# lidongyv/Explicit-Context-Mapping-for-Stereo-Matching

Measured on AMD Instinct MI355X. Metric: stereo-pairs/sec (cmfsm train step fwd+bwd+Adam), higher is better.
Workload: dtype f32; 1 GPU; SceneFlow 960x540 (padded to 576) D=192 batch=4/GPU fwd+bwd+Adam (train.py path); arch=cmfsm, global_batch=4, parallelism=dp1, cost_volume=collapsed into class-indexed 2-D convolutions, launch=eager

## Files before the change

### explicit-context-mapping-for-stereo-matching_amd/csrc/conv3d_wgrad.hip

```cpp
#include "common.h"

#ifdef WG_PROFILE
__device__ unsigned long long wg_prof[4 * 8];
#define WG_T(i) do { const unsigned long long now_ = clock64(); prof[i] += now_ - last; last = now_; } while (0)
#else
#define WG_T(i) do { } while (0)
#endif

namespace {

typedef float f32x16 __attribute__((ext_vector_type(16)));

constexpr int CT = 32;
constexpr int TWV = 16;

template <int STRIDE, int TD, int TH, int KD, int KH = 3, int KW = 3, int DIL = 1>
struct WgCfg {
    static_assert(KD == 1 || (KH == 3 && KW == 3 && DIL == 1), "3-D layers are 3x3x3, dilation 1");
    static constexpr int NTAPS = KH * KW * KD, PADD = KD / 2;
    static constexpr int TG = NTAPS >= 15 ? 4 : NTAPS >= 2 ? 2 : 1, KG = 4 / TG, MAXNT = (NTAPS + TG - 1) / TG;
    static constexpr int ID = (TD - 1) * STRIDE + KD, IH = (TH - 1) * STRIDE + (KH - 1) * DIL + 1,
                         IW = (TWV - 1) * STRIDE + (KW - 1) * DIL + 1;
    static constexpr int RS = IW;
    static constexpr int XCH = ID * IH * RS;
    static constexpr int XSTR = (XCH % 2 == 0) ? XCH + 1 : XCH + 2;
    static constexpr int NV = TD * TH * TWV;
    static constexpr int GSTR = NV + 1;
    static constexpr int LDS_FLOATS = CT * XSTR + CT * GSTR;
    static constexpr int LDS_BYTES = LDS_FLOATS * 4;
};


template <int STRIDE, int TD, int TH, int KD, int KH, int KW, int DIL, int TGI, int KGI, int NLOADS, class Issue>
__device__ __forceinline__ void wg_tile(const float* __restrict__ ga, const float* __restrict__ xb,
                                        f32x16 (&acc)[WgCfg<STRIDE, TD, TH, KD, KH, KW, DIL>::MAXNT], Issue&& issue) {
    using Cfg = WgCfg<STRIDE, TD, TH, KD, KH, KW, DIL>;
    constexpr int IH = Cfg::IH, RS = Cfg::RS;
    constexpr int T0 = TGI * Cfg::MAXNT;
    constexpr int NT = (T0 + Cfg::MAXNT <= Cfg::NTAPS) ? Cfg::MAXNT : Cfg::NTAPS - T0;
    static_assert(NT >= 1, "every wave owns at least one tap");
    constexpr int KSA = TD * TH * TWV / 2;
    constexpr int KS0 = KGI * (KSA / Cfg::KG), KS = KS0 + KSA / Cfg::KG;
    constexpr int KSI = (KS - KS0) * 3 / 4;
    constexpr int LPK = (NLOADS + KSI - 1) / KSI;
    auto b_off = [](int ks, int t) constexpr {
        const int xx = (ks * 2) % TWV, hy = ((ks * 2) / TWV) % TH, dz = (ks * 2) / (TWV * TH);
        const int tap = T0 + t, kd = KD == 3 ? tap / 9 : 0, kh = (tap / KW) % KH, kw = tap % KW;
        return ((dz * STRIDE + kd) * IH + hy * STRIDE + kh * DIL) * RS + xx * STRIDE + kw * DIL;
    };
    float a_cur = ga[KS0 * 2], b_cur[NT];
#pragma unroll
    for (int t = 0; t < NT; ++t) b_cur[t] = xb[b_off(KS0, t)];
#pragma unroll
    for (int ks = KS0; ks < KS; ++ks) {
        float a_nxt = 0.f, b_nxt[NT];
        if (ks + 1 < KS) {
            a_nxt = ga[(ks + 1) * 2];
#pragma unroll
            for (int t = 0; t < NT; ++t) b_nxt[t] = xb[b_off(ks + 1, t)];
        }
#pragma unroll
        for (int q = 0; q < LPK; ++q)
            if ((ks - KS0) * LPK + q < NLOADS) issue((ks - KS0) * LPK + q);
#pragma unroll
        for (int t = 0; t < NT; ++t) acc[t] = __builtin_amdgcn_mfma_f32_32x32x2f32(a_cur, b_cur[t], acc[t], 0, 0, 0);
        __builtin_amdgcn_sched_barrier(0);
        a_cur = a_nxt;
#pragma unroll
        for (int t = 0; t < NT; ++t) b_cur[t] = b_nxt[t];
    }
}

template <int TD, int TH, int KD, int I, int NLOADS, class Issue>
__device__ __forceinline__ void wg_tile_wino(const float* __restrict__ gaw, const float* __restrict__ xbw,
                                             f32x16 (&acc)[4 * KD], Issue&& issue) {
    using Cfg = WgCfg<1, TD, TH, KD>;
    constexpr int IH = Cfg::IH, RS = Cfg::RS, NP = TD + KD - 1;
    constexpr int PAIRS = TWV / 4, KS = (TH / 2) * PAIRS;
    constexpr int RA = I == 0 ? 0 : I == 2 ? 2 : 1, RB = I == 0 ? 2 : I == 1 ? 2 : I == 2 ? 1 : 3;
    float xr_[NP][2][4], gr_[TD][2][2];
    float bq[NP][4], aq[TD][4];
    auto read_raw = [&](int ks) {
        const int tr = ks / PAIRS, pr = ks % PAIRS;
        const float* xk = xbw + 2 * tr * RS + 4 * pr;
        const float* gk = gaw + 2 * tr * TWV + 4 * pr;
#pragma unroll
        for (int p = 0; p < NP; ++p)
#pragma unroll
            for (int j = 0; j < 4; ++j) {
                xr_[p][0][j] = xk[(p * IH + RA) * RS + j];
                xr_[p][1][j] = xk[(p * IH + RB) * RS + j];
            }
#pragma unroll
        for (int d = 0; d < TD; ++d)
#pragma unroll
            for (int r = 0; r < 2; ++r)
#pragma unroll
                for (int c = 0; c < 2; ++c) gr_[d][r][c] = gk[(d * TH + r) * TWV + c];
    };
    auto make_operands = [&]() {
#pragma unroll
        for (int p = 0; p < NP; ++p) {
            float e[4];
#pragma unroll
            for (int j = 0; j < 4; ++j) e[j] = I == 1 ? xr_[p][0][j] + xr_[p][1][j] : xr_[p][0][j] - xr_[p][1][j];
            bq[p][0] = e[0] - e[2]; bq[p][1] = e[1] + e[2]; bq[p][2] = e[2] - e[1]; bq[p][3] = e[1] - e[3];
        }
#pragma unroll
        for (int d = 0; d < TD; ++d) {
            float m[2];
#pragma unroll
            for (int c = 0; c < 2; ++c)
                m[c] = I == 0 ? gr_[d][0][c] : I == 1 ? gr_[d][0][c] + gr_[d][1][c]
                     : I == 2 ? gr_[d][0][c] - gr_[d][1][c] : -gr_[d][1][c];
            aq[d][0] = m[0]; aq[d][1] = m[0] + m[1]; aq[d][2] = m[0] - m[1]; aq[d][3] = -m[1];
        }
    };
    constexpr int NPH = KD == 1 ? 16 : 8, KPP = KS / NPH, LPP = (NLOADS + NPH - 2) / (NPH - 1);
    constexpr int KUNROLL = KD == 1 ? 8 : 1;
    static_assert(KS % NPH == 0, "k-steps split into phases");
    read_raw(0);
    make_operands();
#pragma unroll
    for (int ph = 0; ph < NPH; ++ph) {
        if (ph < NPH - 1) {
#pragma unroll
            for (int q = 0; q < LPP; ++q)
                if (ph * LPP + q < NLOADS) issue(ph * LPP + q);
        }
#pragma unroll KUNROLL
        for (int ks = ph * KPP; ks < (ph + 1) * KPP; ++ks) {
            if (ks + 1 < KS) read_raw(ks + 1);
            __builtin_amdgcn_sched_barrier(0);
#pragma unroll
            for (int j = 0; j < 4; ++j)
#pragma unroll
                for (int kd = 0; kd < KD; ++kd)
#pragma unroll
                    for (int d = 0; d < TD; ++d)
                        acc[j * KD + kd] = __builtin_amdgcn_mfma_f32_32x32x2f32(aq[d][j], bq[d + kd][j], acc[j * KD + kd], 0, 0, 0);
            __builtin_amdgcn_sched_barrier(0);
            if (ks + 1 < KS) make_operands();
            __builtin_amdgcn_sched_barrier(0);
        }
    }
}

template <int STRIDE, int TD, int TH, int KD, int KH = 3, int KW = 3, int DIL = 1, bool WINO = false>
__global__ __launch_bounds__(256, KD == 3 ? 1 : 2) void conv3d_wgrad_mfma(const float* __restrict__ x, const float* __restrict__ gy,
                                                         float* __restrict__ partial, int B, int Ci, int Co, int D,
                                                         int H, int W, int Do, int Ho, int Wo, int tiles_d, int tiles_h,
                                                         int tiles_w, int ci_tiles, int pad_top, int pad_left) {
    using Cfg = WgCfg<STRIDE, TD, TH, KD, KH, KW, DIL>;
    constexpr int ID = Cfg::ID, IH = Cfg::IH, IW = Cfg::IW, XSTR = Cfg::XSTR, NV = Cfg::NV, GSTR = Cfg::GSTR,
                  NTAPS = Cfg::NTAPS, MAXNT = Cfg::MAXNT;
    extern __shared__ __attribute__((aligned(16))) float smem[];
    float* Xs = smem;
    float* Gs = smem + CT * XSTR;

    const int tid = threadIdx.x, lane = tid & 63, wave = tid >> 6;
    const int l31 = lane & 31, half = lane >> 5;
    const int ci0 = (blockIdx.y % ci_tiles) * CT, co0 = (blockIdx.y / ci_tiles) * CT;
    const int tgi = wave % Cfg::TG, kgi = wave / Cfg::TG;
    const int t0 = tgi * MAXNT;
    constexpr int NACC = WINO ? 4 * KD : MAXNT;
    static_assert(!WINO || (STRIDE == 1 && KH == 3 && KW == 3 && DIL == 1 && TH % 2 == 0), "Winograd form: 3x3, stride 1");
    f32x16 acc[NACC];
#pragma unroll
    for (int t = 0; t < NACC; ++t)
#pragma unroll
        for (int i = 0; i < 16; ++i) acc[t][i] = 0.f;

    const size_t HWi = (size_t)H * W, DHWi = (size_t)D * HWi;
    const size_t HWo = (size_t)Ho * Wo, DHWo = (size_t)Do * HWo;
    const int ntiles = B * tiles_d * tiles_h * tiles_w;

    constexpr int NPOSX = ID * IH * IW;
    constexpr int PPX = (NPOSX + 255) / 256;
    constexpr int GPL = 256 / NV;
    static_assert(256 % NV == 0 && CT % GPL == 0, "gy tile must divide the workgroup");
    constexpr int NGRP = CT / GPL;
    constexpr int NLOADS = CT * PPX + NGRP;
    float xr[CT * PPX], gr[NGRP];
    const unsigned xplane = (unsigned)DHWi * 4u, gplane = (unsigned)DHWo * 4u;
    const int nci = Ci - ci0 < CT ? Ci - ci0 : CT, nco = Co - co0 < CT ? Co - co0 : CT;
    unsigned xoff[PPX], goff;
    auto xrs = __builtin_amdgcn_make_buffer_rsrc(const_cast<float*>(x), 0, 0, 0x00020000);
    auto grs = xrs;
    int pdz[PPX], phy[PPX], pxx[PPX], prel[PPX];
#pragma unroll
    for (int j = 0; j < PPX; ++j) {
        int t = tid + j * 256;
        pxx[j] = t % IW; t /= IW;
        phy[j] = t % IH;
        const bool in_tile = tid + j * 256 < NPOSX;
        prel[j] = in_tile ? (t / IH) * (int)HWi + phy[j] * W + pxx[j] : 0;
        pdz[j] = in_tile ? t / IH : -(1 << 20);
    }
    const int gv = tid % NV, gccl = tid / NV;
    const int gxx = gv % TWV, ghy = (gv / TWV) % TH, gdz = gv / (TWV * TH);
    const int grel = gdz * (int)HWo + ghy * Wo + gxx;
    auto prefetch_setup = [&](unsigned tile) {
        const bool live = tile < (unsigned)ntiles;
        unsigned r = live ? tile : 0u;
        const int td = (int)(r % (unsigned)tiles_d); r /= (unsigned)tiles_d;
        const int tw = (int)(r % (unsigned)tiles_w); r /= (unsigned)tiles_w;
        const int th = (int)(r % (unsigned)tiles_h);
        const int b = (int)(r / (unsigned)tiles_h);
        const int od0 = td * TD, oh0 = th * TH, ow0 = tw * TWV;
        const int id0 = od0 * STRIDE - Cfg::PADD, ih0 = oh0 * STRIDE - pad_top, iw0 = ow0 * STRIDE - pad_left;
        const int xbase = id0 * (int)HWi + ih0 * W + iw0;
#pragma unroll
        for (int j = 0; j < PPX; ++j) {
            const bool ok = live && (unsigned)(id0 + pdz[j]) < (unsigned)D && (unsigned)(ih0 + phy[j]) < (unsigned)H &&
                            (unsigned)(iw0 + pxx[j]) < (unsigned)W;
            xoff[j] = ok ? (unsigned)(xbase + prel[j]) * 4u : 0x80000000u;
        }
        xrs = __builtin_amdgcn_make_buffer_rsrc(const_cast<float*>(x + ((size_t)b * Ci + ci0) * DHWi), 0,
                                                (unsigned)nci * xplane, 0x00020000);
        const bool vok = live && od0 + gdz < Do && oh0 + ghy < Ho && ow0 + gxx < Wo;
        goff = vok ? (unsigned)(od0 * (int)HWo + oh0 * Wo + ow0 + grel) * 4u + (unsigned)gccl * gplane : 0x80000000u;
        grs = __builtin_amdgcn_make_buffer_rsrc(const_cast<float*>(gy + ((size_t)b * Co + co0) * DHWo), 0,
                                                (unsigned)nco * gplane, 0x00020000);
    };
    auto prefetch_issue = [&](int i) {
        if (i < CT * PPX) {
            const int cc = i / PPX, j = i % PPX;
            xr[i] = __builtin_bit_cast(float, __builtin_amdgcn_raw_buffer_load_b32(xrs, xoff[j] + (unsigned)cc * xplane, 0, 0));
        } else {
            const int g = i - CT * PPX;
            gr[g] = __builtin_bit_cast(float, __builtin_amdgcn_raw_buffer_load_b32(grs, goff + (unsigned)(g * GPL) * gplane, 0, 0));
        }
    };
#ifdef WG_PROFILE
    unsigned long long prof[8] = {0, 0, 0, 0, 0, 0, 0, 0}, last = clock64();
#endif
    unsigned tile0 = blockIdx.x, tile_end = (unsigned)ntiles, tile_step = gridDim.x;
    if ((gridDim.x & 7u) == 0u) {
        const unsigned xcd = blockIdx.x & 7u, q = (unsigned)ntiles >> 3, rr = (unsigned)ntiles & 7u;
        const unsigned start = xcd * q + (xcd < rr ? xcd : rr);
        tile0 = start + (blockIdx.x >> 3);
        tile_end = start + q + (xcd < rr ? 1u : 0u);
        tile_step = gridDim.x >> 3;
    }
    prefetch_setup(tile0 < tile_end ? tile0 : (unsigned)ntiles);
#pragma unroll
    for (int i = 0; i < NLOADS; ++i) prefetch_issue(i);
    WG_T(0);
    for (unsigned tile = tile0; tile < tile_end; tile += tile_step) {
        __syncthreads();
        WG_T(1);
#pragma unroll
        for (int j = 0; j < PPX; ++j) {
            const int p = tid + j * 256 < NPOSX ? tid + j * 256 : NPOSX;
#pragma unroll
            for (int cc = 0; cc < CT; ++cc) Xs[cc * XSTR + p] = xr[cc * PPX + j];
        }
#pragma unroll
        for (int g = 0; g < NGRP; ++g) Gs[(g * GPL + tid / NV) * GSTR + tid % NV] = gr[g];
        WG_T(2);
        __syncthreads();
        WG_T(3);
        prefetch_setup(tile + tile_step < tile_end ? tile + tile_step : (unsigned)ntiles);
        WG_T(4);
        if constexpr (WINO) {
            const float* gaw = Gs + l31 * GSTR + half * 2;
            const float* xbw = Xs + l31 * XSTR + half * 2;
            switch (wave) {
                case 0: wg_tile_wino<TD, TH, KD, 0, NLOADS>(gaw, xbw, acc, prefetch_issue); break;
                case 1: wg_tile_wino<TD, TH, KD, 1, NLOADS>(gaw, xbw, acc, prefetch_issue); break;
                case 2: wg_tile_wino<TD, TH, KD, 2, NLOADS>(gaw, xbw, acc, prefetch_issue); break;
                default: wg_tile_wino<TD, TH, KD, 3, NLOADS>(gaw, xbw, acc, prefetch_issue); break;
            }
        } else {
        const float* ga = Gs + l31 * GSTR + half;
        const float* xb = Xs + l31 * XSTR + half * STRIDE;
        switch (wave) {
            case 0: wg_tile<STRIDE, TD, TH, KD, KH, KW, DIL, 0 % Cfg::TG, 0 / Cfg::TG, NLOADS>(ga, xb, acc, prefetch_issue); break;
            case 1: wg_tile<STRIDE, TD, TH, KD, KH, KW, DIL, 1 % Cfg::TG, 1 / Cfg::TG, NLOADS>(ga, xb, acc, prefetch_issue); break;
            case 2: wg_tile<STRIDE, TD, TH, KD, KH, KW, DIL, 2 % Cfg::TG, 2 / Cfg::TG, NLOADS>(ga, xb, acc, prefetch_issue); break;
            default: wg_tile<STRIDE, TD, TH, KD, KH, KW, DIL, 3 % Cfg::TG, 3 / Cfg::TG, NLOADS>(ga, xb, acc, prefetch_issue); break;
        }
        }
        WG_T(5);
    }
#ifdef WG_PROFILE
    if (blockIdx.x == 0 && blockIdx.y == 0 && lane == 0)
        for (int i = 0; i < 8; ++i) wg_prof[wave * 8 + i] = prof[i];
#endif
    if constexpr (WINO) {
        float* pw = partial + (size_t)blockIdx.x * 16 * KD * Co * Ci;
        const int ci = ci0 + l31;
#pragma unroll
        for (int t = 0; t < NACC; ++t) {
            const int j = t / KD, kd = t % KD;
#pragma unroll
            for (int i = 0; i < 16; ++i) {
                const int co = co0 + mfma32_row(i, half);
                if (co < Co && ci < Ci) pw[((size_t)((wave * 4 + j) * KD + kd) * Co + co) * Ci + ci] = acc[t][i];
            }
        }
        return;
    }
    float* pp = partial + ((size_t)blockIdx.x * Cfg::KG + kgi) * Co * Ci * NTAPS;
#pragma unroll
    for (int t = 0; t < MAXNT; ++t) {
        const int tap = t0 + t;
        if (tap >= NTAPS) continue;
        const int ci = ci0 + l31;
#pragma unroll
        for (int i = 0; i < 16; ++i) {
            const int co = co0 + mfma32_row(i, half);
            if (co < Co && ci < Ci) pp[((size_t)co * Ci + ci) * NTAPS + tap] = acc[t][i];
        }
    }
}

__global__ __launch_bounds__(256) void wgrad_reduce(const float* __restrict__ partial, float* __restrict__ gw, int n, int P) {
    __shared__ float sm[8][32];
    const int o = threadIdx.x & 31, grp = threadIdx.x >> 5;
    const int i = blockIdx.x * 32 + o;
    float s = 0.f;
    if (i < n) {
        float s0 = 0.f, s1 = 0.f, s2 = 0.f, s3 = 0.f;
        int p = grp;
        for (; p + 24 < P; p += 32) {
            s0 += partial[(size_t)p * n + i];
            s1 += partial[(size_t)(p + 8) * n + i];
            s2 += partial[(size_t)(p + 16) * n + i];
            s3 += partial[(size_t)(p + 24) * n + i];
        }
        for (; p < P; p += 8) s0 += partial[(size_t)p * n + i];
        s = (s0 + s1) + (s2 + s3);
    }
    sm[grp][o] = s;
    __syncthreads();
    if (grp == 0 && i < n) {
        float t = 0.f;
#pragma unroll
        for (int g = 0; g < 8; ++g) t += sm[g][o];
        gw[i] = t;
    }
}

__global__ void wgrad_wino_finish(const float* __restrict__ gU, float* __restrict__ gw, int Co, int Ci, int KD) {
    const int idx = blockIdx.x * blockDim.x + threadIdx.x;
    if (idx >= Co * Ci * KD) return;
    const int kd = idx % KD, ci = (idx / KD) % Ci, co = idx / (KD * Ci);
    float u[4][4];
#pragma unroll
    for (int i = 0; i < 4; ++i)
#pragma unroll
        for (int j = 0; j < 4; ++j) u[i][j] = gU[((size_t)((i * 4 + j) * KD + kd) * Co + co) * Ci + ci];
    float t[3][4];
#pragma unroll
    for (int j = 0; j < 4; ++j) {
        t[0][j] = u[0][j] + 0.5f * (u[1][j] + u[2][j]);
        t[1][j] = 0.5f * (u[1][j] - u[2][j]);
        t[2][j] = 0.5f * (u[1][j] + u[2][j]) + u[3][j];
    }
    float* o = gw + (((size_t)co * Ci + ci) * KD + kd) * 9;
#pragma unroll
    for (int a = 0; a < 3; ++a) {
        o[a * 3 + 0] = t[a][0] + 0.5f * (t[a][1] + t[a][2]);
        o[a * 3 + 1] = 0.5f * (t[a][1] - t[a][2]);
        o[a * 3 + 2] = 0.5f * (t[a][1] + t[a][2]) + t[a][3];
    }
}

inline int wgrad_workers(int Ci, int Co, long long ntiles, int occ = 1) {
    const int ytiles = ((Ci + CT - 1) / CT) * ((Co + CT - 1) / CT);
    long long p = 256 * occ / ytiles;
    if (p < 1) p = 1;
    if (p > ntiles) p = ntiles;
    return (int)p;
}

template <int STRIDE, int TD, int TH, int KD, int KH = 3, int KW = 3, int DIL = 1>
int launch_wgrad(const float* x, const float* gy, float* gw, float* partial, int B, int Ci, int Co, int D, int H, int W,
                 hipStream_t st, int Ho = 0, int Wo = 0, int pad_top = 1, int pad_left = 1) {
    using Cfg = WgCfg<STRIDE, TD, TH, KD, KH, KW, DIL>;
    const int Do = (D - 1) / STRIDE + 1;
    if (Ho <= 0) Ho = (H - 1) / STRIDE + 1;
    if (Wo <= 0) Wo = (W - 1) / STRIDE + 1;
    const int tiles_d = (Do + TD - 1) / TD, tiles_h = (Ho + TH - 1) / TH, tiles_w = (Wo + TWV - 1) / TWV;
    const long long ntiles = (long long)B * tiles_d * tiles_h * tiles_w;
    const int ci_tiles = (Ci + CT - 1) / CT, co_tiles = (Co + CT - 1) / CT;
    const int P = wgrad_workers(Ci, Co, ntiles, KD == 3 ? 1 : 2);
    auto kern = conv3d_wgrad_mfma<STRIDE, TD, TH, KD, KH, KW, DIL>;
    {
        const hipError_t e = ecm_allow_lds(reinterpret_cast<const void*>(kern), Cfg::LDS_BYTES);
        if (e != hipSuccess) return (int)e;
    }
    hipLaunchKernelGGL(kern, dim3(P, ci_tiles * co_tiles), dim3(256), Cfg::LDS_BYTES, st, x, gy, partial, B, Ci, Co, D, H,
                       W, Do, Ho, Wo, tiles_d, tiles_h, tiles_w, ci_tiles, pad_top, pad_left);
    const int n = Co * Ci * Cfg::NTAPS;
    hipLaunchKernelGGL(wgrad_reduce, dim3((n + 31) / 32), dim3(256), 0, st, partial, gw, n, P * Cfg::KG);
    return ECM_LAUNCH_RESULT();
}

template <int TD, int TH, int KD>
int launch_wgrad_wino(const float* x, const float* gy, float* gw, float* scratch, int B, int Ci, int Co, int D, int H, int W,
                      hipStream_t st) {
    using Cfg = WgCfg<1, TD, TH, KD>;
    const int tiles_d = (D + TD - 1) / TD, tiles_h = (H + TH - 1) / TH, tiles_w = (W + TWV - 1) / TWV;
    const long long ntiles = (long long)B * tiles_d * tiles_h * tiles_w;
    const int ci_tiles = (Ci + CT - 1) / CT, co_tiles = (Co + CT - 1) / CT;
    const int P = wgrad_workers(Ci, Co, ntiles, KD == 3 ? 1 : 2);
    auto kern = conv3d_wgrad_mfma<1, TD, TH, KD, 3, 3, 1, true>;
    {
        const hipError_t e = ecm_allow_lds(reinterpret_cast<const void*>(kern), Cfg::LDS_BYTES);
        if (e != hipSuccess) return (int)e;
    }
    const int n = 16 * KD * Co * Ci;
    float* partial = scratch;
    float* gU = scratch + (size_t)P * n;
    hipLaunchKernelGGL(kern, dim3(P, ci_tiles * co_tiles), dim3(256), Cfg::LDS_BYTES, st, x, gy, partial, B, Ci, Co, D, H,
                       W, D, H, W, tiles_d, tiles_h, tiles_w, ci_tiles, 1, 1);
    hipLaunchKernelGGL(wgrad_reduce, dim3((n + 31) / 32), dim3(256), 0, st, partial, gU, n, P);
    hipLaunchKernelGGL(wgrad_wino_finish, dim3((Co * Ci * KD + 255) / 256), dim3(256), 0, st, gU, gw, Co, Ci, KD);
    return ECM_LAUNCH_RESULT();
}

inline long long ntiles_wino(int B, int D, int H, int W, int kd) {
    const int TD = kd == 3 ? 2 : 1, TH = kd == 3 ? 8 : 16;
    return (long long)B * ((D + TD - 1) / TD) * ((H + TH - 1) / TH) * ((W + TWV - 1) / TWV);
}

inline long long ntiles_for(int B, int D, int H, int W, int stride) {
    const int Do = (D - 1) / stride + 1, Ho = (H - 1) / stride + 1, Wo = (W - 1) / stride + 1;
    const int TD = stride == 1 ? 2 : 1, TH = stride == 1 ? 8 : 4;
    return (long long)B * ((Do + TD - 1) / TD) * ((Ho + TH - 1) / TH) * ((Wo + TWV - 1) / TWV);
}

}

extern "C" long long ecm_conv3d_wgrad_scratch_bytes(int B, int Ci, int Co, int D, int H, int W, int stride) {
    if (B <= 0 || Ci <= 0 || Co <= 0 || D <= 0 || H <= 0 || W <= 0 || (stride != 1 && stride != 2)) return 0;
    return (long long)wgrad_workers(Ci, Co, ntiles_for(B, D, H, W, stride)) * Co * Ci * 27 * (long long)sizeof(float);
}

extern "C" int ecm_conv3d_k3_wgrad(const float* x, const float* gy, float* gw, void* scratch, long long scratch_bytes,
                                   int B, int Ci, int Co, int D, int H, int W, int stride, void* stream) {
    ECM_CHECK_ARG(x && gy && gw && scratch && B > 0 && Ci > 0 && Co > 0 && D > 0 && H > 0 && W > 0);
    if (stride != 1 && stride != 2) return ECM_EUNSUP;
    if ((long long)D * H * W * 4 * 32 >= 0x7fffffffLL) return ECM_EUNSUP;
    if (ntiles_for(B, D, H, W, stride) >= 0x7fffffffLL) return ECM_EUNSUP;
    if (scratch_bytes < ecm_conv3d_wgrad_scratch_bytes(B, Ci, Co, D, H, W, stride)) return ECM_ESCRATCH;
    float* partial = static_cast<float*>(scratch);
    hipStream_t st = ecm_stream(stream);
    if (stride == 1) return launch_wgrad<1, 2, 8, 3>(x, gy, gw, partial, B, Ci, Co, D, H, W, st);
    return launch_wgrad<2, 1, 4, 3>(x, gy, gw, partial, B, Ci, Co, D, H, W, st);
}

namespace {
inline long long ntiles2d_ex(int B, int Ho, int Wo, int stride) {
    const int th = stride == 1 ? 16 : 8;
    return (long long)B * ((Ho + th - 1) / th) * ((Wo + TWV - 1) / TWV);
}
}

extern "C" long long ecm_conv2d_wgrad_ex_scratch_bytes(int B, int Ci, int Co, int Ho, int Wo, int kh, int kw, int stride) {
    if (B <= 0 || Ci <= 0 || Co <= 0 || Ho <= 0 || Wo <= 0 || kh <= 0 || kw <= 0) return 0;
    return (long long)wgrad_workers(Ci, Co, ntiles2d_ex(B, Ho, Wo, stride), 2) * 4 * Co * Ci * kh * kw * (long long)sizeof(float);
}

extern "C" int ecm_conv2d_wgrad_ex(const float* x, const float* gy, float* gw, void* scratch, long long scratch_bytes, int B,
                                   int Ci, int Co, int H, int W, int kh, int kw, int stride, int dil, int pad_top,
                                   int pad_left, int Ho, int Wo, void* stream) {
    ECM_CHECK_ARG(x && gy && gw && scratch && B > 0 && Ci > 0 && Co > 0 && H > 0 && W > 0 && Ho > 0 && Wo > 0);
    if ((long long)H * W * 4 * 32 >= 0x7fffffffLL || (long long)Ho * Wo * 4 * 32 >= 0x7fffffffLL) return ECM_EUNSUP;
    if (ntiles2d_ex(B, Ho, Wo, stride) >= 0x7fffffffLL) return ECM_EUNSUP;
    if (scratch_bytes < ecm_conv2d_wgrad_ex_scratch_bytes(B, Ci, Co, Ho, Wo, kh, kw, stride)) return ECM_ESCRATCH;
    float* partial = static_cast<float*>(scratch);
    hipStream_t st = ecm_stream(stream);
#define WG2(KH, KW, S, DL, TH) if (kh == KH && kw == KW && stride == S && dil == DL) \
        return launch_wgrad<S, 1, TH, 1, KH, KW, DL>(x, gy, gw, partial, B, Ci, Co, 1, H, W, st, Ho, Wo, pad_top, pad_left)
    WG2(3, 3, 1, 1, 16);
    WG2(3, 3, 1, 2, 16);
    WG2(3, 3, 1, 4, 16);
    WG2(3, 3, 2, 1, 8);
    WG2(3, 5, 1, 1, 16);
    WG2(1, 1, 1, 1, 16);
    WG2(1, 1, 2, 1, 8);
#undef WG2
    return ECM_EUNSUP;
}

extern "C" long long ecm_conv_wino_wgrad_scratch_bytes(int B, int Ci, int Co, int D, int H, int W, int kd) {
    if (B <= 0 || Ci <= 0 || Co <= 0 || D <= 0 || H <= 0 || W <= 0 || (kd != 1 && kd != 3)) return 0;
    const long long P = wgrad_workers(Ci, Co, ntiles_wino(B, D, H, W, kd), kd == 3 ? 1 : 2);
    return (P + 1) * 16LL * kd * Co * Ci * (long long)sizeof(float);
}

extern "C" int ecm_conv_wino_wgrad(const float* x, const float* gy, float* gw, void* scratch, long long scratch_bytes, int B,
                                   int Ci, int Co, int D, int H, int W, int kd, void* stream) {
    ECM_CHECK_ARG(x && gy && gw && scratch && B > 0 && Ci > 0 && Co > 0 && D > 0 && H > 0 && W > 0);
    if (kd != 1 && kd != 3) return ECM_EUNSUP;
    if ((long long)D * H * W * 4 * 32 >= 0x7fffffffLL || ntiles_wino(B, D, H, W, kd) >= 0x7fffffffLL) return ECM_EUNSUP;
    if (scratch_bytes < ecm_conv_wino_wgrad_scratch_bytes(B, Ci, Co, D, H, W, kd)) return ECM_ESCRATCH;
    hipStream_t st = ecm_stream(stream);
    if (kd == 3) return launch_wgrad_wino<2, 8, 3>(x, gy, gw, static_cast<float*>(scratch), B, Ci, Co, D, H, W, st);
    return launch_wgrad_wino<1, 16, 1>(x, gy, gw, static_cast<float*>(scratch), B, Ci, Co, D, H, W, st);
}
```

Baseline: 32.67 pairs/s.

## Add direct MFMA weight-gradient kernel for few-channel stem conv

Adds a dedicated direct (non-Winograd) weight-gradient kernel for 2-D 3x3 convolutions with at most 3 input and 32 output channels, such as the image stem. It uses MFMA 32x32x2 over an im2col-like LDS layout, register-prefetches the next tile, and reduces per-block partials with a persistent grid of up to 512 workers. The aim is to avoid the Winograd path's transform overhead and poor channel utilization when Ci is tiny. Columns beyond Ci*9 are wasted in the MFMA, and scratch sizing is adjusted to cover both paths.

```diff
diff --git a/explicit-context-mapping-for-stereo-matching_amd/csrc/conv3d_wgrad.hip b/explicit-context-mapping-for-stereo-matching_amd/csrc/conv3d_wgrad.hip
--- a/explicit-context-mapping-for-stereo-matching_amd/csrc/conv3d_wgrad.hip
+++ b/explicit-context-mapping-for-stereo-matching_amd/csrc/conv3d_wgrad.hip
@@ -433,6 +433,133 @@
     return (long long)B * ((Do + TD - 1) / TD) * ((Ho + TH - 1) / TH) * ((Wo + TWV - 1) / TWV);
 }
 
+constexpr int STH = 8, STW = 64, SNV = STH * STW;
+constexpr int SGSTR = SNV + 1;
+constexpr int SRS = 67, SPS = 681;
+constexpr int SNH = (STH + 2) * (STW + 2);
+constexpr int S_LDS_BYTES = (32 * SGSTR + 3 * SPS) * 4;
+static_assert((STH + 1) * SRS + STW + 2 <= SPS, "channel stride too small");
+static_assert(4 * 1024 <= 32 * SGSTR, "the end-of-kernel reduction reuses the gy image");
+
+__global__ __launch_bounds__(256) void conv2d_stem_wgrad(const float* __restrict__ x, const float* __restrict__ gy,
+                                                         float* __restrict__ partial, int B, int Ci, int Co, int D, int H, int W,
+                                                         int tiles_h, int tiles_w) {
+    extern __shared__ __attribute__((aligned(16))) float smem[];
+    float* Ys = smem;
+    float* Xs = smem + 32 * SGSTR;
+    float* Ps = Ys;
+    const int tid = threadIdx.x, lane = tid & 63, wave = tid >> 6, l31 = lane & 31, half = lane >> 5;
+    const size_t HW = (size_t)H * W, DHW = (size_t)D * HW;
+    const int ncol = Ci * 9;
+    const int col = l31 < ncol ? l31 : 0;
+    const int toff = (col / 9) * SPS + ((col / 3) % 3) * SRS + col % 3;
+    f32x16 acc;
+#pragma unroll
+    for (int i = 0; i < 16; ++i) acc[i] = 0.f;
+    const unsigned plane = (unsigned)DHW * 4u;
+    const int ntiles = B * D * tiles_h * tiles_w;
+    constexpr int PX = (SNH + 255) / 256;
+    float yr[64], xr[3][PX];
+    int xdst[PX];
+#pragma unroll
+    for (int j = 0; j < PX; ++j) {
+        const int e = tid + j * 256;
+        xdst[j] = e < SNH ? (e / (STW + 2)) * SRS + e % (STW + 2) : -1;
+    }
+    auto prefetch = [&](unsigned tile) {
+        const bool live = tile < (unsigned)ntiles;
+        unsigned r = live ? tile : 0u;
+        const int tw = (int)(r % (unsigned)tiles_w); r /= (unsigned)tiles_w;
+        const int th = (int)(r % (unsigned)tiles_h); r /= (unsigned)tiles_h;
+        const int d = (int)(r % (unsigned)D);
+        const int b = (int)(r / (unsigned)D);
+        const int h0 = th * STH, w0 = tw * STW;
+        const unsigned dbase = (unsigned)d * (unsigned)HW;
+        unsigned off[2];
+#pragma unroll
+        for (int j = 0; j < 2; ++j) {
+            const int v = tid + j * 256;
+            const int gh = h0 + v / STW, gw_ = w0 + v % STW;
+            off[j] = (live && gh < H && gw_ < W) ? (dbase + (unsigned)(gh * W + gw_)) * 4u : 0x80000000u;
+        }
+        const auto yrs = __builtin_amdgcn_make_buffer_rsrc(const_cast<float*>(gy + (size_t)b * Co * DHW), 0,
+                                                           (unsigned)Co * plane, 0x00020000);
+#pragma unroll
+        for (int cc = 0; cc < 32; ++cc)
+#pragma unroll
+            for (int j = 0; j < 2; ++j)
+                yr[cc * 2 + j] = __builtin_bit_cast(
+                    float, __builtin_amdgcn_raw_buffer_load_b32(yrs, off[j] + (unsigned)cc * plane, 0, 0));
+        const auto xrs = __builtin_amdgcn_make_buffer_rsrc(const_cast<float*>(x + (size_t)b * Ci * DHW), 0,
+                                                           (unsigned)Ci * plane, 0x00020000);
+#pragma unroll
+        for (int j = 0; j < PX; ++j) {
+            const int e = tid + j * 256;
+            const int gh = h0 - 1 + e / (STW + 2), gw_ = w0 - 1 + e % (STW + 2);
+            const bool ok = live && e < SNH && (unsigned)gh < (unsigned)H && (unsigned)gw_ < (unsigned)W;
+            const unsigned o = ok ? (dbase + (unsigned)(gh * W + gw_)) * 4u : 0x80000000u;
+#pragma unroll
+            for (int c = 0; c < 3; ++c)
+                xr[c][j] = __builtin_bit_cast(float, __builtin_amdgcn_raw_buffer_load_b32(xrs, o + (unsigned)c * plane, 0, 0));
+        }
+    };
+    prefetch(blockIdx.x);
+    for (unsigned tile = blockIdx.x; tile < (unsigned)ntiles; tile += gridDim.x) {
+        __syncthreads();
+#pragma unroll
+        for (int cc = 0; cc < 32; ++cc)
+#pragma unroll
+            for (int j = 0; j < 2; ++j) Ys[cc * SGSTR + tid + j * 256] = yr[cc * 2 + j];
+#pragma unroll
+        for (int j = 0; j < PX; ++j)
+            if (xdst[j] >= 0) {
+#pragma unroll
+                for (int c = 0; c < 3; ++c) Xs[c * SPS + xdst[j]] = xr[c][j];
+            }
+        __syncthreads();
+        prefetch(tile + gridDim.x);
+        const float* ya = Ys + l31 * SGSTR + half;
+        const float* xb = Xs + toff + half;
+#pragma unroll
+        for (int rr = 0; rr < STH / 4; ++rr) {
+            const int hy = wave + rr * 4;
+#pragma unroll 8
+            for (int xx = 0; xx < STW; xx += 2) {
+                const float a = ya[hy * STW + xx];
+                const float bv = l31 < ncol ? xb[hy * SRS + xx] : 0.f;
+                acc = __builtin_amdgcn_mfma_f32_32x32x2f32(a, bv, acc, 0, 0, 0);
+            }
+        }
+    }
+    __syncthreads();
+#pragma unroll
+    for (int i = 0; i < 16; ++i) Ps[wave * 1024 + mfma32_row(i, half) * 32 + l31] = acc[i];
+    __syncthreads();
+    for (int e = tid; e < 1024; e += 256) {
+        const int co = e >> 5, t = e & 31;
+        if (t < ncol && co < Co)
+            partial[(size_t)blockIdx.x * Co * ncol + co * ncol + t] = (Ps[e] + Ps[1024 + e]) + (Ps[2048 + e] + Ps[3072 + e]);
+    }
+}
+
+inline bool stem_wgrad_ok(int Ci, int Co, int kd) { return kd == 1 && Ci <= 3 && Co <= 32; }
+inline long long stem_tiles(int B, int D, int H, int W) { return (long long)B * D * ((H + STH - 1) / STH) * ((W + STW - 1) / STW); }
+inline int stem_workers(long long ntiles) { return (int)(ntiles < 512 ? ntiles : 512); }
+
+int launch_stem_wgrad(const float* x, const float* gy, float* gw, float* partial, int B, int Ci, int Co, int D, int H, int W,
+                      hipStream_t st) {
+    const int P = stem_workers(stem_tiles(B, D, H, W));
+    {
+        const hipError_t e = ecm_allow_lds(reinterpret_cast<const void*>(conv2d_stem_wgrad), S_LDS_BYTES);
+        if (e != hipSuccess) return (int)e;
+    }
+    hipLaunchKernelGGL(conv2d_stem_wgrad, dim3(P), dim3(256), S_LDS_BYTES, st, x, gy, partial, B, Ci, Co, D, H, W,
+                       (H + STH - 1) / STH, (W + STW - 1) / STW);
+    const int n = Co * Ci * 9;
+    hipLaunchKernelGGL(wgrad_reduce, dim3((n + 31) / 32), dim3(256), 0, st, partial, gw, n, P);
+    return ECM_LAUNCH_RESULT();
+}
+
 }
 
 extern "C" long long ecm_conv3d_wgrad_scratch_bytes(int B, int Ci, int Co, int D, int H, int W, int stride) {
@@ -490,7 +617,10 @@
 extern "C" long long ecm_conv_wino_wgrad_scratch_bytes(int B, int Ci, int Co, int D, int H, int W, int kd) {
     if (B <= 0 || Ci <= 0 || Co <= 0 || D <= 0 || H <= 0 || W <= 0 || (kd != 1 && kd != 3)) return 0;
     const long long P = wgrad_workers(Ci, Co, ntiles_wino(B, D, H, W, kd), kd == 3 ? 1 : 2);
-    return (P + 1) * 16LL * kd * Co * Ci * (long long)sizeof(float);
+    const long long wino = (P + 1) * 16LL * kd * Co * Ci * (long long)sizeof(float);
+    if (!stem_wgrad_ok(Ci, Co, kd)) return wino;
+    const long long direct = (long long)stem_workers(stem_tiles(B, D, H, W)) * Co * Ci * 9 * (long long)sizeof(float);
+    return direct > wino ? direct : wino;
 }
 
 extern "C" int ecm_conv_wino_wgrad(const float* x, const float* gy, float* gw, void* scratch, long long scratch_bytes, int B,
@@ -500,6 +630,8 @@
     if ((long long)D * H * W * 4 * 32 >= 0x7fffffffLL || ntiles_wino(B, D, H, W, kd) >= 0x7fffffffLL) return ECM_EUNSUP;
     if (scratch_bytes < ecm_conv_wino_wgrad_scratch_bytes(B, Ci, Co, D, H, W, kd)) return ECM_ESCRATCH;
     hipStream_t st = ecm_stream(stream);
+    if (stem_wgrad_ok(Ci, Co, kd) && stem_tiles(B, D, H, W) < 0x7fffffffLL)
+        return launch_stem_wgrad(x, gy, gw, static_cast<float*>(scratch), B, Ci, Co, D, H, W, st);
     if (kd == 3) return launch_wgrad_wino<2, 8, 3>(x, gy, gw, static_cast<float*>(scratch), B, Ci, Co, D, H, W, st);
     return launch_wgrad_wino<1, 16, 1>(x, gy, gw, static_cast<float*>(scratch), B, Ci, Co, D, H, W, st);
 }
```

Result: no change. 32.58 pairs/s (-0.3%).
